# musyoku/wavenet

Hardware: AMD Instinct MI355X
Metric: audio samples/sec: train fwd+bwd, 4x10-layer dilated stack (cfg2) (higher is better)
Workload: dtype f32 storage+accumulate / fp16x2 split products (2^-21)

## Files before the change

wavenet_amd/csrc/mfma_gemm_b3.hip:

```cpp
#include "mfma_gemm.hpp"
#include "split_w.hpp"
#include "h2_ops.hpp"
#include <type_traits>

namespace wn {

template <bool WMAX>
__global__ void k_split_w(CGArgs a, int mode, int mtiles, int chunks_per_src, __bf16* __restrict__ img, int one) {
    if (WMAX) {
        const float mw = split_w_tile<true>(a, mode, mtiles, chunks_per_src, img, one, (int)blockIdx.x, 1.f);
        if (threadIdx.x == 0) atomicMax(const_cast<unsigned*>(a.wmax_dev), __float_as_uint(mw));
    } else {
        split_w_tile<false>(a, mode, mtiles, chunks_per_src, img, one, (int)blockIdx.x, one == 3 ? h2_scale(a.wmax_dev, kH2ScaleW) : 1.f);
    }
}

__device__ __forceinline__ int b3_ch(int r, int h) { return (r & 3) + 8 * (r >> 2) + 4 * h; }

struct RowMap { long long row[4]; bool ok[4]; };

__device__ __forceinline__ RowMap row_map(long long no, bool nvalid, int lane) {
    RowMap m;
#pragma unroll
    for (int it = 0; it < 4; ++it) {
// ... 421 lines not shown
    if (MODE == 3) {
        const bool live = rbase - a.off >= a.gate_Z;
#pragma unroll
        for (int pr = 0; pr < MT / 2; ++pr) {
            if (t0 + 2 * pr >= mtiles) break;
            const int col = ((t0 >> 1) + pr) * 32;
            float4 tf[4], ts[4], tz[4];
#pragma unroll
            for (int q = 0; q < 4; ++q) {
                float f4[4], s4[4];
#pragma unroll
                for (int e = 0; e < 4; ++e) {
                    f4[e] = fast_tanh(live ? acc[2 * pr][4 * q + e] : 0.f);
                    s4[e] = fast_sigmoid(live ? acc[2 * pr + 1][4 * q + e] : 0.f);
                }
                tf[q] = make_float4(f4[0], f4[1], f4[2], f4[3]);
                ts[q] = make_float4(s4[0], s4[1], s4[2], s4[3]);
                tz[q] = make_float4(f4[0] * s4[0], f4[1] * s4[1], f4[2] * s4[2], f4[3] * s4[3]);
            }
            tile_store_rows(patch, lane, tz, a.gate_z, a.M, col, rm);
            if (a.gate_f) {
                tile_store_rows(patch, lane, tf, a.gate_f, a.M, col, rm);
                tile_store_rows(patch, lane, ts, a.gate_s, a.M, col, rm);
            }
        }
        return;
    }
    if (MODE == 4) {
        const bool live = rbase - a.off >= a.gate_Z;
#pragma unroll
        for (int mt = 0; mt < MT; ++mt) {
            if (t0 + mt >= mtiles) break;
            const int col = (t0 + mt) * 32;
            float4 vf[4], vs[4], vr[4], tf[4], ts[4], tr[4], da[4], dg[4];
            rows_load(a.gate_f, a.M, col, rm, lane, vf);
            rows_load(a.gate_s, a.M, col, rm, lane, vs);
            if (a.residual) rows_load(a.residual, a.M, col, rm, lane, vr);
            rows_to_tile(patch, lane, vf, tf);
            rows_to_tile(patch, lane, vs, ts);
            if (a.residual) rows_to_tile(patch, lane, vr, tr);
#pragma unroll
            for (int q = 0; q < 4; ++q) {
                float4 dz = make_float4(acc[mt][4 * q], acc[mt][4 * q + 1], acc[mt][4 * q + 2], acc[mt][4 * q + 3]);
                if (a.residual) { dz.x += tr[q].x; dz.y += tr[q].y; dz.z += tr[q].z; dz.w += tr[q].w; }
                if (!live) dz = make_float4(0.f, 0.f, 0.f, 0.f);
                const float4 f4 = tf[q], s4 = ts[q];
                da[q] = make_float4(dz.x * s4.x * (1.f - f4.x * f4.x), dz.y * s4.y * (1.f - f4.y * f4.y),
                                    dz.z * s4.z * (1.f - f4.z * f4.z), dz.w * s4.w * (1.f - f4.w * f4.w));
                dg[q] = make_float4(dz.x * f4.x * s4.x * (1.f - s4.x), dz.y * f4.y * s4.y * (1.f - s4.y),
                                    dz.z * f4.z * s4.z * (1.f - s4.z), dz.w * f4.w * s4.w * (1.f - s4.w));
            }
            tile_store_rows(patch, lane, da, a.gate_z, 2 * a.M, col, rm);
            tile_store_rows(patch, lane, dg, a.gate_z, 2 * a.M, a.M + col, rm);
        }
        return;
    }
    float omax = 0.f;
#pragma unroll
    for (int mt = 0; mt < MT; ++mt) {
        if (t0 + mt >= mtiles) break;
        float* __restrict__ og = (MODE == 2) ? a.out[t0 + mt] : a.out[0];
        const int col = (MODE == 2) ? 0 : (t0 + mt) * 32;
        float4 t[4], v[4], u[4];
#pragma unroll
        for (int q = 0; q < 4; ++q) t[q] = make_float4(acc[mt][4 * q], acc[mt][4 * q + 1], acc[mt][4 * q + 2], acc[mt][4 * q + 3]);
        if (MODE == 0 && a.gate_x) {
            rows_load(a.gate_x, a.ldo, col, rm, lane, v);
            rows_to_tile(patch, lane, v, u);
#pragma unroll
            for (int q = 0; q < 4; ++q) {
                t[q].x *= act_grad(u[q].x, a.gate_act); t[q].y *= act_grad(u[q].y, a.gate_act);
                t[q].z *= act_grad(u[q].z, a.gate_act); t[q].w *= act_grad(u[q].w, a.gate_act);
            }
        }
        if (MODE == 0 && a.residual) {
            rows_load(a.residual, a.ldo, col, rm, lane, v);
            rows_to_tile(patch, lane, v, u);
#pragma unroll
            for (int q = 0; q < 4; ++q) { t[q].x += u[q].x; t[q].y += u[q].y; t[q].z += u[q].z; t[q].w += u[q].w; }
        }
        if (a.accumulate) {
            rows_load(og, a.ldo, col, rm, lane, v);
            rows_to_tile(patch, lane, v, u);
#pragma unroll
            for (int q = 0; q < 4; ++q) { t[q].x += u[q].x; t[q].y += u[q].y; t[q].z += u[q].z; t[q].w += u[q].w; }
        }
        if (MODE == 0 && a.outmax_dev && nvalid) {
#pragma unroll
            for (int q = 0; q < 4; ++q)
                omax = fmaxf(omax, fmaxf(fmaxf(fabsf(t[q].x), fabsf(t[q].y)), fmaxf(fabsf(t[q].z), fabsf(t[q].w))));
        }
        tile_store_rows(patch, lane, t, og, a.ldo, col, rm);
    }
    if (MODE == 0 && a.outmax_dev) {
        for (int o = 32; o >= 1; o >>= 1) omax = fmaxf(omax, __shfl_xor(omax, o));
        if (lane == 0) {
            const unsigned bits = __float_as_uint(omax);
            if (bits > __hip_atomic_load(a.outmax_dev, __ATOMIC_RELAXED, __HIP_MEMORY_SCOPE_AGENT)) atomicMax(a.outmax_dev, bits);
        }
    }
}

typedef float f32x4 __attribute__((ext_vector_type(4)));
__device__ __forceinline__ void asm_load16(f32x4& dst, const float* p) {
    asm volatile("global_load_dwordx4 %0, %1, off" : "=v"(dst) : "v"(p) : "memory");
}
static constexpr int kH2qTB = kTileBytes * 2 / 3;
static constexpr int kH2qHalf = kH2qTB / 2;
static constexpr int kH2qLds = 4 * 8 * kH2qHalf;

__device__ __forceinline__ void asm_load16s(f32x4& dst, unsigned voff, const char* sbase) {
    asm volatile("global_load_dwordx4 %0, %1, %2" : "=v"(dst) : "v"(voff), "s"(sbase) : "memory");
}
__device__ __forceinline__ void asm_dma2(unsigned voff, const char* sbase, unsigned m0v) {
    asm volatile("s_mov_b32 m0, %2\n\ts_nop 0\n\tglobal_load_lds_dwordx4 %0, %1\n\tglobal_load_lds_dwordx4 %0, %1 offset:1024"
                 :: "v"(voff), "s"(sbase), "s"(m0v) : "memory", "m0");
}

template <int MODE, int ACT>
__global__ __launch_bounds__(256, 2) void k_colgemm_h2q(CGArgs a, const __bf16* __restrict__ img, int mtiles, int nchunks,
                                                        long long x_stride) {
    constexpr int MT = 8;
    static_assert(MODE == 0 || MODE == 2, "plain contractions only");
    extern __shared__ __attribute__((aligned(16))) char ldsq[];
    const float h2sx = h2_scale(a.xmax_dev, kH2ScaleX);
    const float h2sw = h2_scale(a.wmax_dev, kH2ScaleW);
    const int tid = threadIdx.x, lane = tid & 63, wave = tid >> 6;
    const int j = lane & 31, h = lane >> 5;
    int bx, by;
    {
        const int ny = (mtiles + MT - 1) / MT;
        const int nx = gridDim.x / ny;
        const int id = blockIdx.x;
        const int full = nx & ~7;
        if (id < full * ny) {
            const int g = id / (8 * ny), rem = id - g * 8 * ny;
            bx = g * 8 + (rem & 7);
            by = rem >> 3;
        } else {
            const int t = id - full * ny;
            by = t % ny;
            bx = full + t / ny;
        }
    }
    const int t0 = by * MT;
    const long long n = ((long long)bx * 4 + wave) * 32 + j;
    const bool nvalid = n < a.N;
    long long rb0 = 0;
    int rbase = -(1 << 30);
    long long no = n;
    if (nvalid) {
        long long b = n / a.rows_out_per_b;
        rbase = (int)(n - b * a.rows_out_per_b) + a.off;
        rb0 = b * a.rows_src_per_b;
        if (a.out_rows_per_b) no = b * a.out_rows_per_b + a.out_row0 + (n - b * a.rows_out_per_b);
    }
    f32x16 acc[MT];
#pragma unroll
    for (int mt = 0; mt < MT; ++mt)
#pragma unroll
        for (int r = 0; r < 16; ++r) acc[mt][r] = 0.f;
    if (MODE == 0) {
        for (int src = 0; src < a.nsrc; ++src)
            if (a.bias[src]) {
#pragma unroll
                for (int mt = 0; mt < MT; ++mt)
                    if (t0 + mt < mtiles) {
#pragma unroll
                        for (int r = 0; r < 16; ++r) acc[mt][r] += a.bias[src][(t0 + mt) * 32 + b3_ch(r, h)] * (h2sw * h2sx);
                    }
            }
    }
    const int nhalf = 2 * nchunks;
    const unsigned lds0 = (unsigned)(unsigned long long)(__attribute__((address_space(3))) char*)ldsq;
    const int swave = __builtin_amdgcn_readfirstlane(wave);
    unsigned tile_off[2];
#pragma unroll
    for (int tt = 0; tt < 2; ++tt)
        tile_off[tt] = (unsigned)((t0 + swave + 4 * tt < mtiles) ? t0 + swave + 4 * tt : mtiles - 1) * kH2qTB + lane * 16;
    const long long img_stride = (long long)mtiles * kH2qTB;
    auto dma_half = [&](int s) {
        const int ss = s < nhalf ? s : nhalf - 1;
        const char* base = reinterpret_cast<const char*>(img) + (long long)(ss >> 1) * img_stride + (ss & 1) * kH2qHalf;
#pragma unroll
        for (int tt = 0; tt < 2; ++tt)
            asm_dma2(tile_off[tt], base, lds0 + ((s & 3) * MT + swave + 4 * tt) * kH2qHalf);
    };
    f32x4 xr[4][2];
    const int rs0 = rbase + a.soff[0];
    const bool rv0 = rs0 >= 0 && rs0 < a.rows_src_per_b;
    const float msk0 = rv0 ? 1.f : 0.f;
    const unsigned x_off = (unsigned)(((rb0 + (rv0 ? rs0 : 0)) * (a.ldx ? a.ldx : a.K[0]) + 8 * h) * 4);
    const char* x0 = reinterpret_cast<const char*>(a.X[0]);
    auto load_x = [&](int s, auto slot_tag) {
        constexpr int slot = decltype(slot_tag)::value;
        const int ss = s < nhalf ? s : nhalf - 1;
        const char* base = x0 + (long long)(ss >> 1) * x_stride + (ss & 1) * 64;
        asm_load16s(xr[slot][0], x_off, base);
        asm_load16s(xr[slot][1], x_off + 16, base);
    };
    f16x8 xh[2], xm[2];
    auto split_one = [&](const f32x4 (&raw)[2], float ms, int e, f16x8& oh, f16x8& om) {
        const float v = raw[e >> 2][e & 3];
        _Float16 a0, a1;
        split2h(act_apply_t<ACT>(v) * (ms * h2sx), a0, a1);
        oh[e] = a0; om[e] = a1;
    };
    using I0 = std::integral_constant<int, 0>;
    using I1 = std::integral_constant<int, 1>;
    using I2 = std::integral_constant<int, 2>;
    using I3 = std::integral_constant<int, 3>;
    load_x(0, I0{});
    asm volatile("s_waitcnt vmcnt(0)" : "+v"(xr[0][0]), "+v"(xr[0][1]) : : "memory");
#pragma unroll
    for (int e = 0; e < 8; ++e) split_one(xr[0], msk0, e, xh[0], xm[0]);
    asm volatile("" : "+v"(xh[0]), "+v"(xm[0]));
    dma_half(0); load_x(1, I1{});
    dma_half(1); load_x(2, I2{});
    dma_half(2); load_x(3, I3{});

    auto step = [&](int s, auto p_tag) {
        constexpr int p = decltype(p_tag)::value;
        constexpr int set = p & 1, nxt = 1 - set;
        constexpr int rn = (p + 1) & 3;
        asm volatile("s_waitcnt vmcnt(12)" : "+v"(xr[rn][0]), "+v"(xr[rn][1]) : : "memory");
        const float ms = msk0;
        asm volatile("s_waitcnt lgkmcnt(0)" ::: "memory");
        __builtin_amdgcn_s_barrier();
        dma_half(s + 3);
        const char* Ab = ldsq + (p * MT) * kH2qHalf + lane * 16;
        f16x8 fr[2][2];
        auto ldA = [&](int mt, f16x8 (&f)[2]) {
            f[0] = *reinterpret_cast<const f16x8*>(Ab + mt * kH2qHalf);
            f[1] = *reinterpret_cast<const f16x8*>(Ab + mt * kH2qHalf + 1024);
        };
        ldA(0, fr[0]);
#pragma unroll
        for (int mt = 0; mt < MT; ++mt) {
            f16x8 (&f)[2] = fr[mt & 1];
            asm volatile("" ::"v"(f[0]));
            asm volatile("" ::"v"(f[1]));
            if (mt + 1 < MT) ldA(mt + 1, fr[(mt + 1) & 1]);
            __builtin_amdgcn_sched_barrier(0);
            split_one(xr[rn], ms, mt, nxt ? xh[1] : xh[0], nxt ? xm[1] : xm[0]);
            acc[mt] = __builtin_amdgcn_mfma_f32_32x32x16_f16(f[1], xh[set], acc[mt], 0, 0, 0);
            acc[mt] = __builtin_amdgcn_mfma_f32_32x32x16_f16(f[0], xm[set], acc[mt], 0, 0, 0);
            acc[mt] = __builtin_amdgcn_mfma_f32_32x32x16_f16(f[0], xh[set], acc[mt], 0, 0, 0);
            __builtin_amdgcn_sched_barrier(0);
        }
        asm volatile("" : "+v"(xh[nxt]), "+v"(xm[nxt]));
        load_x(s + 4, p_tag);
    };
    for (int s = 0; s < nhalf; s += 4) {
        step(s, I0{});
        step(s + 1, I1{});
        step(s + 2, I2{});
        step(s + 3, I3{});
    }
    asm volatile("s_waitcnt vmcnt(0)"
                 : "+v"(xr[0][0]), "+v"(xr[0][1]), "+v"(xr[1][0]), "+v"(xr[1][1]), "+v"(xr[2][0]), "+v"(xr[2][1]),
                   "+v"(xr[3][0]), "+v"(xr[3][1])
                 :
                 : "memory");
#pragma unroll
    for (int mt = 0; mt < MT; ++mt)
#pragma unroll
        for (int r = 0; r < 16; ++r) acc[mt][r] *= 1.f / (h2sw * h2sx);
    __syncthreads();
    float* patch = reinterpret_cast<float*>(ldsq) + wave * 1024;
    const RowMap rm = row_map(no, nvalid, lane);
#pragma unroll
    for (int mt = 0; mt < MT; ++mt) {
        if (t0 + mt >= mtiles) break;
        float* __restrict__ og = (MODE == 2) ? a.out[t0 + mt] : a.out[0];
        const int col = (MODE == 2) ? 0 : (t0 + mt) * 32;
        float4 t[4], v[4], u[4];
#pragma unroll
        for (int q = 0; q < 4; ++q) t[q] = make_float4(acc[mt][4 * q], acc[mt][4 * q + 1], acc[mt][4 * q + 2], acc[mt][4 * q + 3]);
        if (MODE == 0 && a.gate_x) {
            rows_load(a.gate_x, a.ldo, col, rm, lane, v);
            rows_to_tile(patch, lane, v, u);
#pragma unroll
            for (int q = 0; q < 4; ++q) {
                t[q].x *= act_grad(u[q].x, a.gate_act); t[q].y *= act_grad(u[q].y, a.gate_act);
                t[q].z *= act_grad(u[q].z, a.gate_act); t[q].w *= act_grad(u[q].w, a.gate_act);
            }
        }
        if (MODE == 0 && a.residual) {
            rows_load(a.residual, a.ldo, col, rm, lane, v);
            rows_to_tile(patch, lane, v, u);
#pragma unroll
            for (int q = 0; q < 4; ++q) { t[q].x += u[q].x; t[q].y += u[q].y; t[q].z += u[q].z; t[q].w += u[q].w; }
        }
        if (a.accumulate) {
            rows_load(og, a.ldo, col, rm, lane, v);
            rows_to_tile(patch, lane, v, u);
#pragma unroll
            for (int q = 0; q < 4; ++q) { t[q].x += u[q].x; t[q].y += u[q].y; t[q].z += u[q].z; t[q].w += u[q].w; }
        }
        tile_store_rows(patch, lane, t, og, a.ldo, col, rm);
    }
}

int launch_colgemm_b3(Call& c, CGArgs& a, int mode, int nprob, hipStream_t s) {
    if (mode != 0 && mode != 2 && mode != 3 && mode != 4 && mode != 5 && mode != 6) return WN_ESHAPE;
    if (mode == 6 && !(c.fp16x2() && a.M == 256 && a.nsrc == 1 && a.xent_target && a.xent_loss && a.out[0] &&
                       cdiv(a.N, 128) <= kXentBlocks))
        return WN_ESHAPE;
    int mtiles, nchunks, cps;
    if (mode == 0 || mode >= 3) {
        if (a.M % 32) return WN_ESHAPE;
        if ((mode == 3 || mode == 5) && a.nsrc > WN_GATE_TAPS) return WN_ESHAPE;
        if (mode == 5 && !(c.one_term() && a.M == 128 && a.ldo == 128)) return WN_ESHAPE;
        for (int i = 0; i < a.nsrc; ++i)
            if (a.K[i] != a.K[0] || a.K[i] % 32) return WN_ESHAPE;
        mtiles = ((mode == 3 || mode == 5) ? 2 : 1) * a.M / 32;
        cps = a.K[0] / 32;
        nchunks = a.nsrc * cps;
    } else {
        if (a.M != 32 || a.K[0] % 32) return WN_ESHAPE;
        mtiles = nprob;
        cps = a.K[0] / 32;
        nchunks = cps;
    }
    const bool one = c.one_term();
    const bool h2 = c.fp16x2() && ((a.h2_ok || a.xmax_dev) && (mode == 0 || mode == 2) || mode == 6);
    const size_t bytes = (size_t)nchunks * mtiles * (one ? kTileBytes / 3 : (h2 ? kTileBytes * 2 / 3 : kTileBytes));
    const size_t bytes2 = mode == 5 ? (size_t)16 * (kTileBytes / 3) : 0;
    const __bf16* pimg = nullptr; const unsigned* pwmax = nullptr;
    const bool planned = plan_split_image(c, a, mode, mtiles, cps, nchunks, one ? 1 : (h2 ? 3 : 0), bytes, &pimg, &pwmax);
    __bf16* img = planned ? const_cast<__bf16*>(pimg)
                          : reinterpret_cast<__bf16*>(c.scratch(bytes + bytes2, "the split weight image"));
    if (!img) return WN_EARG;
    if (planned) {
        a.wmax_dev = pwmax;
    } else {
    if (h2) {
        bool fresh = false;
        unsigned* wm = c.word(reinterpret_cast<const char*>(a.W[0]) + (((unsigned)mode & 7u) << 8 | ((unsigned)a.nsrc & 255u)), &fresh, s);
        if (!wm) return WN_EARG;
        a.wmax_dev = wm;
        if (fresh) hipLaunchKernelGGL(k_split_w<true>, dim3(nchunks * mtiles), dim3(256), 0, s, a, mode, mtiles, cps, img, 3);
    }
    hipLaunchKernelGGL(k_split_w<false>, dim3(nchunks * mtiles), dim3(256), 0, s, a, mode, mtiles, cps, img, one ? 1 : (h2 ? 3 : 0));
    }
    if (mode == 5) {
        if (!a.proj_W || !a.residual || !a.gate_z || a.act != WN_ACT_NONE || mtiles != 8) {
            wn::set_error("colgemm_b3: fused-layer mode needs Wp, the residual input, z and 128 gate channels");
            return WN_EARG;
        }
        CGArgs b{};
        b.nsrc = 1; b.W[0] = a.proj_W; b.wsm[0] = 128; b.wsk = 1; b.K[0] = 128; b.M = 128;
        __bf16* img2 = reinterpret_cast<__bf16*>(reinterpret_cast<char*>(img) + bytes);
        hipLaunchKernelGGL(k_split_w<false>, dim3(16), dim3(256), 0, s, b, 0, 4, 4, img2, 1);
        hipLaunchKernelGGL((k_colgemm_b3<5, WN_ACT_NONE, 1, 8>), dim3(cdiv(a.N, 128)), dim3(256), 0, s, a,
                           (const __bf16*)img, mtiles, nchunks, cps, (const __bf16*)img2);
        WN_LAUNCH_CHECK();
        return WN_OK;
    }
    const bool mt8 = (one || h2) && mtiles >= 8;
    dim3 grid(cdiv(a.N, 128) * cdiv(mtiles, mt8 ? 8 : 4));
    if (mode == 6) {
#define X_LAUNCH(ACT_, ROWS_) hipLaunchKernelGGL((k_colgemm_b3<6, ACT_, 3, 8, ROWS_>), grid, dim3(256), 0, s, a, (const __bf16*)img, \
                                                 mtiles, nchunks, cps, (const __bf16*)nullptr)
        if (c.flag(WN_EXEC_HEAD_ROW_NLL)) {
            if (a.act == WN_ACT_RELU) X_LAUNCH(WN_ACT_RELU, true);
            else if (a.act == WN_ACT_ELU) X_LAUNCH(WN_ACT_ELU, true);
            else X_LAUNCH(WN_ACT_NONE, true);
        } else if (a.act == WN_ACT_RELU) X_LAUNCH(WN_ACT_RELU, false);
        else if (a.act == WN_ACT_ELU) X_LAUNCH(WN_ACT_ELU, false);
        else X_LAUNCH(WN_ACT_NONE, false);
#undef X_LAUNCH
        WN_LAUNCH_CHECK();
        return WN_OK;
    }
#define CG_LAUNCH(MODE_, ACT_)                                                                                          \
    do {                                                                                                                \
        if (mt8) hipLaunchKernelGGL((k_colgemm_b3<MODE_, ACT_, 1, 8>), grid, dim3(256), 0, s, a, (const __bf16*)img,    \
                                    mtiles, nchunks, cps, (const __bf16*)nullptr);                                      \
        else if (one) hipLaunchKernelGGL((k_colgemm_b3<MODE_, ACT_, 1, 4>), grid, dim3(256), 0, s, a,                   \
                                         (const __bf16*)img, mtiles, nchunks, cps, (const __bf16*)nullptr);             \
        else hipLaunchKernelGGL((k_colgemm_b3<MODE_, ACT_, 6, 4>), grid, dim3(256), 0, s, a, (const __bf16*)img,        \
                                mtiles, nchunks, cps, (const __bf16*)nullptr);                                          \
    } while (0)
#define CG_LAUNCH_H2(MODE_, ACT_)                                                                                       \
    do {                                                                                                                \
        if (mt8) hipLaunchKernelGGL((k_colgemm_b3<MODE_, ACT_, 3, 8>), grid, dim3(256), 0, s, a, (const __bf16*)img,    \
                                    mtiles, nchunks, cps, (const __bf16*)nullptr);                                      \
        else hipLaunchKernelGGL((k_colgemm_b3<MODE_, ACT_, 3, 4>), grid, dim3(256), 0, s, a, (const __bf16*)img,        \
                                mtiles, nchunks, cps, (const __bf16*)nullptr);                                          \
    } while (0)
    long long x_stride = 128;
    bool lean = h2 && mt8 && mode == 0 && (nchunks & 1) == 0 && !c.flag(WN_EXEC_NO_PIPELINED_GEMM) &&
                (a.N / a.rows_out_per_b + 1) * (long long)a.rows_src_per_b * (a.ldx ? a.ldx : a.K[0]) * 4 < (1ll << 32);
    if (lean && mode == 0 && a.nsrc > 1) {
        x_stride = (const char*)a.X[1] - (const char*)a.X[0];
        lean = cps == 1;
        for (int i = 1; i < a.nsrc && lean; ++i)
            lean = a.soff[i] == a.soff[0] && a.K[i] == a.K[0] && (const char*)a.X[i] - (const char*)a.X[i - 1] == x_stride;
    } else if (lean && mode == 0) {
        lean = a.nsrc == 1;
    }
    if (lean) {
        WN_MAX_LDS_ONCE(kH2qLds, k_colgemm_h2q<0, WN_ACT_NONE>, k_colgemm_h2q<0, WN_ACT_RELU>, k_colgemm_h2q<0, WN_ACT_ELU>);
#define Q_LAUNCH(MODE_, ACT_)                                                                                 \
    hipLaunchKernelGGL((k_colgemm_h2q<MODE_, ACT_>), grid, dim3(256), kH2qLds, s, a, (const __bf16*)img, mtiles, nchunks, x_stride)
        if (a.act == WN_ACT_RELU) Q_LAUNCH(0, WN_ACT_RELU);
        else if (a.act == WN_ACT_ELU) Q_LAUNCH(0, WN_ACT_ELU);
        else Q_LAUNCH(0, WN_ACT_NONE);
#undef Q_LAUNCH
        WN_LAUNCH_CHECK();
        return WN_OK;
    }
    if (h2) {
        if (mode == 2) CG_LAUNCH_H2(2, WN_ACT_NONE);
        else if (a.act == WN_ACT_RELU) CG_LAUNCH_H2(0, WN_ACT_RELU);
        else if (a.act == WN_ACT_ELU) CG_LAUNCH_H2(0, WN_ACT_ELU);
        else CG_LAUNCH_H2(0, WN_ACT_NONE);
        WN_LAUNCH_CHECK();
        return WN_OK;
    }
#undef CG_LAUNCH_H2
    if (mode == 3) {
        if (a.act != WN_ACT_NONE || !a.gate_z) { wn::set_error("colgemm_b3: gate mode takes no activation and needs gate_z"); return WN_EARG; }
        CG_LAUNCH(3, WN_ACT_NONE);
    } else if (mode == 4) {
        if (a.act != WN_ACT_NONE || !a.gate_z || !a.gate_f || !a.gate_s) { wn::set_error("colgemm_b3: gate-backward mode needs f, s and the output"); return WN_EARG; }
        CG_LAUNCH(4, WN_ACT_NONE);
    } else if (mode == 0) {
        if (a.outmax_dev) plan_xmax_written(c, a.out[0]);
        if (a.act == WN_ACT_RELU) CG_LAUNCH(0, WN_ACT_RELU);
        else if (a.act == WN_ACT_ELU) CG_LAUNCH(0, WN_ACT_ELU);
        else if (a.act == WN_ACT_NONE) CG_LAUNCH(0, WN_ACT_NONE);
        else { wn::set_error("colgemm_b3: unknown activation %d", a.act); return WN_EARG; }
    } else {
        if (a.act != WN_ACT_NONE) { wn::set_error("colgemm_b3: multi-problem mode takes no activation"); return WN_EARG; }
        CG_LAUNCH(2, WN_ACT_NONE);
    }
#undef CG_LAUNCH
    WN_LAUNCH_CHECK();
    return WN_OK;
}

template <int MT, bool HAS_B2, int ACT, bool ONE>
__global__ __launch_bounds__(256, 2) void k_wgrad_b3(WGArgs a) {
    __shared__ __attribute__((aligned(16))) char lds[MT * kTileBytes];
    constexpr int NF = MT / 2 > 0 ? MT / 2 : 1;
    const int tid = threadIdx.x, lane = tid & 63, wv = tid >> 6;
    const int j = lane & 31, h = lane >> 5;
    const int p = blockIdx.y * 4 + wv;
    const bool active = p < a.nprob;
    const int m0 = blockIdx.z * (MT * 32);
    const int b = blockIdx.x / a.wgs_per_b;
    const int r_begin = (blockIdx.x - b * a.wgs_per_b) * a.rows_per_wg;
    const int r_end = min(a.rows_A_per_b, r_begin + a.rows_per_wg);
    const float* __restrict__ Ab = a.A + ((long long)b * a.rows_A_per_b) * a.lda + m0;
    const float* __restrict__ Bb = a.Bp[active ? p : 0] + ((long long)b * a.rows_B_per_b + a.off) * a.ldb + j;
    const float* __restrict__ B2b = a.B2p[active ? p : 0] ? a.B2p[active ? p : 0] + ((long long)b * a.rows_B_per_b + a.off) * a.ldb + j : nullptr;
    f32x16 acc[MT];
#pragma unroll
    for (int mt = 0; mt < MT; ++mt)
#pragma unroll
        for (int r = 0; r < 16; ++r) acc[mt][r] = 0.f;

    float ar[NF][8], br[2][8], b2r[2][8];
    const float* __restrict__ B2s = HAS_B2 ? B2b : Bb;
    const float amask = active ? 1.f : 0.f;
    int fm[NF], fg[NF];
#pragma unroll
    for (int it = 0; it < NF; ++it) {
        const int f = it * 256 + tid;
        fm[it] = f % (MT * 32);
        fg[it] = f / (MT * 32);
    }
    auto issue = [&](int r0) {
        const bool full = r0 + 32 <= r_end && r0 + a.off >= 0 && r0 + 31 + a.off < a.rows_B_per_b;
        if (full) {
#pragma unroll
            for (int it = 0; it < NF; ++it) {
                const float* ap = Ab + (long long)(r0 + 8 * (fg[it] & 3)) * a.lda + fm[it];
#pragma unroll
                for (int jj = 0; jj < 8; ++jj) ar[it][jj] = ap[(long long)jj * a.lda];
            }
            const float* bp = Bb + (long long)(r0 + 8 * h) * a.ldb;
            const float* b2p = B2s + (long long)(r0 + 8 * h) * a.ldb;
#pragma unroll
            for (int ks = 0; ks < 2; ++ks)
#pragma unroll
                for (int jj = 0; jj < 8; ++jj) {
                    br[ks][jj] = bp[(long long)(16 * ks + jj) * a.ldb];
                    if (HAS_B2) b2r[ks][jj] = b2p[(long long)(16 * ks + jj) * a.ldb];
                }
            return;
        }
#pragma unroll
        for (int it = 0; it < NF; ++it)
#pragma unroll
            for (int jj = 0; jj < 8; ++jj) {
                const int r = r0 + 8 * (fg[it] & 3) + jj;
                const int rc = r < r_end ? r : r_end - 1;
                ar[it][jj] = Ab[(long long)rc * a.lda + fm[it]];
            }
#pragma unroll
        for (int ks = 0; ks < 2; ++ks)
#pragma unroll
            for (int jj = 0; jj < 8; ++jj) {
                const int r = r0 + 16 * ks + 8 * h + jj;
                int rc = r < r_end ? r : r_end - 1;
                if (rc + a.off < 0) rc = -a.off;
                if (rc + a.off >= a.rows_B_per_b) rc = a.rows_B_per_b - 1 - a.off;
                br[ks][jj] = Bb[(long long)rc * a.ldb];
                if (HAS_B2) b2r[ks][jj] = B2s[(long long)rc * a.ldb];
            }
    };
    if (r_begin < r_end) issue(r_begin);
    for (int r0 = r_begin; r0 < r_end; r0 += 32) {
        bf16x8 ah[NF], am[NF], al[NF], bh[2], bm[2], bl[2];
        const bool edge = !(r0 + 32 <= r_end && r0 + a.off >= 0 && r0 + 31 + a.off < a.rows_B_per_b);
#pragma unroll
        for (int it = 0; it < NF; ++it)
#pragma unroll
            for (int e = 0; e < 8; ++e) {
                float av = ar[it][e];
                if (edge) av *= (r0 + 8 * (fg[it] & 3) + e) < r_end ? 1.f : 0.f;
                __bf16 x0, x1, x2;
                split3(av, x0, x1, x2);
                ah[it][e] = x0; am[it][e] = x1; al[it][e] = x2;
            }
#pragma unroll
        for (int ks = 0; ks < 2; ++ks)
#pragma unroll
            for (int e = 0; e < 8; ++e) {
                float bv = act_apply_t<ACT>(br[ks][e]) * amask;
                if (HAS_B2) bv *= b2r[ks][e];
                if (edge) {
                    const int rb = r0 + 16 * ks + 8 * h + e;
                    bv *= (rb < r_end && rb + a.off >= 0 && rb + a.off < a.rows_B_per_b) ? 1.f : 0.f;
                }
                __bf16 x0, x1, x2;
                split3(bv, x0, x1, x2);
                bh[ks][e] = x0; bm[ks][e] = x1; bl[ks][e] = x2;
            }
        __syncthreads();
#pragma unroll
        for (int it = 0; it < NF; ++it) {
            const int f = it * 256 + tid;
            const int m = f % (MT * 32), g = f / (MT * 32);
            if (MT >= 2 || g < 4) {
                char* d = lds + (m >> 5) * kTileBytes + ((g >> 1) * 3) * 1024 + ((m & 31) + 32 * (g & 1)) * 16;
                *reinterpret_cast<bf16x8*>(d) = ah[it];
                *reinterpret_cast<bf16x8*>(d + 1024) = am[it];
                *reinterpret_cast<bf16x8*>(d + 2048) = al[it];
            }
        }
        __syncthreads();
        if (r0 + 32 < r_end) issue(r0 + 32);
        const char* Al = lds + lane * 16;
#pragma unroll
        for (int mt = 0; mt < MT; ++mt) {
#pragma unroll
            for (int ks = 0; ks < 2; ++ks) {
                const char* q = Al + mt * kTileBytes + ks * 3 * 1024;
                const bf16x8 xh = *reinterpret_cast<const bf16x8*>(q);
                const bf16x8 xm = *reinterpret_cast<const bf16x8*>(q + 1024);
                const bf16x8 xl = *reinterpret_cast<const bf16x8*>(q + 2048);
                if (!ONE) {
                    acc[mt] = __builtin_amdgcn_mfma_f32_32x32x16_bf16(xl, bh[ks], acc[mt], 0, 0, 0);
                    acc[mt] = __builtin_amdgcn_mfma_f32_32x32x16_bf16(xh, bl[ks], acc[mt], 0, 0, 0);
                    acc[mt] = __builtin_amdgcn_mfma_f32_32x32x16_bf16(xm, bm[ks], acc[mt], 0, 0, 0);
                    acc[mt] = __builtin_amdgcn_mfma_f32_32x32x16_bf16(xm, bh[ks], acc[mt], 0, 0, 0);
                    acc[mt] = __builtin_amdgcn_mfma_f32_32x32x16_bf16(xh, bm[ks], acc[mt], 0, 0, 0);
                }
                acc[mt] = __builtin_amdgcn_mfma_f32_32x32x16_bf16(xh, bh[ks], acc[mt], 0, 0, 0);
            }
        }
    }
    if (!active) return;
    if (a.fixed_part) {
        const long long M = (long long)gridDim.z * (MT * 32);
        float* __restrict__ q = a.fixed_part + (((long long)blockIdx.x * a.nprob + p) * M) * 32 + j;
#pragma unroll
        for (int mt = 0; mt < MT; ++mt)
#pragma unroll
            for (int r = 0; r < 16; ++r) q[(long long)(m0 + mt * 32 + b3_ch(r, h)) * 32] = acc[mt][r];
        return;
    }
    float* __restrict__ o = a.out[p];
#pragma unroll
    for (int mt = 0; mt < MT; ++mt)
#pragma unroll
        for (int r = 0; r < 16; ++r)
            atomicAdd(o + (long long)(m0 + mt * 32 + b3_ch(r, h)) * a.ldo + (long long)j * (a.osk ? a.osk : 1), acc[mt][r]);
}

template <bool HAS_B2, int ACT, int TM>
__global__ __launch_bounds__(512, 1) void k_wgrad_b3w(WGArgs a) {
    constexpr int MT = 8;
    constexpr bool ONE = TM == 1;
    constexpr bool H2 = TM == 3;
    const float h2sa = H2 ? h2_scale(a.amax_dev, 1.f) : 1.f;
    const float h2sb = H2 ? h2_scale(a.bmax_dev, kH2ScaleX) : 1.f;
    extern __shared__ __attribute__((aligned(16))) char ldsw[];
    const int tid = threadIdx.x, lane = tid & 63, wv = tid >> 6;
    const int j = lane & 31, h = lane >> 5;
    const int p = blockIdx.y * 8 + wv;
    const bool active = p < a.nprob;
    const int off = a.off + a.offp[active ? p : 0];
    const int b = blockIdx.x / a.wgs_per_b;
    const int r_begin = (blockIdx.x - b * a.wgs_per_b) * a.rows_per_wg;
    const int r_end = min(a.rows_A_per_b, r_begin + a.rows_per_wg);
    const float* __restrict__ Ab = a.A + ((long long)b * a.rows_A_per_b) * a.lda;
    const float* __restrict__ Bb = a.Bp[active ? p : 0] + ((long long)b * a.rows_B_per_b + off) * a.ldb + j;
    const float* __restrict__ B2b = a.B2p[active ? p : 0] ? a.B2p[active ? p : 0] + ((long long)b * a.rows_B_per_b + off) * a.ldb + j : nullptr;
    f32x16 acc[MT];
#pragma unroll
    for (int mt = 0; mt < MT; ++mt)
#pragma unroll
        for (int r = 0; r < 16; ++r) acc[mt][r] = 0.f;

    const int fm = tid & 255;
    const int fhh = tid >> 8;
    float ar[2][8], br[2][8], b2r[2][8];
    const float* __restrict__ B2s = HAS_B2 ? B2b : Bb;
    auto issue = [&](int r0) {
        const bool full = r0 + 32 <= r_end && r0 + off >= 0 && r0 + 31 + off < a.rows_B_per_b;
        if (full) {
#pragma unroll
            for (int ks = 0; ks < 2; ++ks) {
                const float* ap = Ab + (long long)(r0 + 16 * ks + 8 * fhh) * a.lda + fm;
#pragma unroll
                for (int jj = 0; jj < 8; ++jj) ar[ks][jj] = ap[(long long)jj * a.lda];
            }
            const float* bp = Bb + (long long)(r0 + 8 * h) * a.ldb;
            const float* b2p = B2s + (long long)(r0 + 8 * h) * a.ldb;
#pragma unroll
            for (int ks = 0; ks < 2; ++ks)
#pragma unroll
                for (int jj = 0; jj < 8; ++jj) {
                    br[ks][jj] = bp[(long long)(16 * ks + jj) * a.ldb];
                    if (HAS_B2) b2r[ks][jj] = b2p[(long long)(16 * ks + jj) * a.ldb];
                }
            return;
        }
#pragma unroll
        for (int ks = 0; ks < 2; ++ks)
#pragma unroll
            for (int jj = 0; jj < 8; ++jj) {
                const int r = r0 + 16 * ks + 8 * fhh + jj;
                const int rc = r < r_end ? r : r_end - 1;
                ar[ks][jj] = Ab[(long long)rc * a.lda + fm];
            }
#pragma unroll
        for (int ks = 0; ks < 2; ++ks)
#pragma unroll
            for (int jj = 0; jj < 8; ++jj) {
                const int r = r0 + 16 * ks + 8 * h + jj;
                int rc = r < r_end ? r : r_end - 1;
                if (rc + off < 0) rc = -off;
                if (rc + off >= a.rows_B_per_b) rc = a.rows_B_per_b - 1 - off;
                br[ks][jj] = Bb[(long long)rc * a.ldb];
                if (HAS_B2) b2r[ks][jj] = B2s[(long long)rc * a.ldb];
// ... 385 lines not shown
```

Measured before the change: 47.53 million.

## Add persistent weight-stationary pipelined kernel for mode-2 fp16x2 dz GEMM

Adds a persistent kernel for the mode-2 fp16x2 GEMM with 8 chunks and ldo 32. Each wave keeps its layer's split weight fragments in registers, and the block walks a contiguous range of 32-column tiles. Within a step it double-buffers the split X tile in LDS and overlaps the next tile's global load, split and store with the current tile's MFMAs. The grid is sized to device occupancy, which aims to cut repeated weight loads and launch and tail overhead. It costs a large register footprint at one block per CU and a more complex schedule built on sched barriers.

```diff
diff --git a/wavenet_amd/csrc/mfma_gemm_b3.hip b/wavenet_amd/csrc/mfma_gemm_b3.hip
--- a/wavenet_amd/csrc/mfma_gemm_b3.hip
+++ b/wavenet_amd/csrc/mfma_gemm_b3.hip
@@ -747,6 +747,185 @@
     }
 }
 
+static constexpr int kWsTile = 32 * 1024;
+static constexpr int kWsLds = 2 * kWsTile + 8 * 4096;
+static constexpr int kWsAhead = 2;
+
+__global__ __launch_bounds__(512, 1) void k_dz_ws(CGArgs a, const __bf16* __restrict__ img, int mtiles, int ntiles, int nranges) {
+    extern __shared__ __attribute__((aligned(16))) char ldsw[];
+    const float h2sx = h2_scale(a.xmax_dev, kH2ScaleX);
+    const float h2sw = h2_scale(a.wmax_dev, kH2ScaleW);
+    const int tid = threadIdx.x, lane = tid & 63;
+    const int wave = __builtin_amdgcn_readfirstlane(tid >> 6);
+    const int j = lane & 31, h = lane >> 5;
+    int range, grp;
+    {
+        const int ng = (mtiles + 7) >> 3;
+        const int id = blockIdx.x;
+        const int full = nranges & ~7;
+        if (id < full * ng) {
+            const int g = id / (8 * ng), rem = id - g * 8 * ng;
+            range = g * 8 + (rem & 7);
+            grp = rem >> 3;
+        } else {
+            const int t = id - full * ng;
+            grp = t % ng;
+            range = full + t / ng;
+        }
+    }
+    const int t_lo = (int)((long long)range * ntiles / nranges), t_hi = (int)((long long)(range + 1) * ntiles / nranges);
+    if (t_lo >= t_hi) return;
+    const int layer = grp * 8 + wave;
+    const bool live = layer < mtiles;
+    const int N = (int)a.N, rows_out = a.rows_out_per_b, rows_src = a.rows_src_per_b, shift = a.off + a.soff[0];
+    const int ldo = a.ldo;
+    const long long ldx = a.ldx ? a.ldx : a.K[0];
+    const float* __restrict__ X = a.X[0];
+    float* __restrict__ og = a.out[live ? layer : 0];
+
+    f16x8 A[16][2];
+    {
+        const char* ip = reinterpret_cast<const char*>(img) + (long long)(live ? layer : mtiles - 1) * kH2qTB + lane * 16;
+#pragma unroll
+        for (int kk = 0; kk < 16; ++kk)
+#pragma unroll
+            for (int pl = 0; pl < 2; ++pl)
+                A[kk][pl] = *reinterpret_cast<const f16x8*>(ip + (long long)(kk >> 1) * mtiles * kH2qTB + (kk & 1) * kH2qHalf + pl * 1024);
+    }
+
+    auto advance = [&](int& n, int& b, int& r, int by) {
+        n += by; r += by;
+        const bool wrap = r >= rows_out;
+        r -= wrap ? rows_out : 0;
+        b += wrap ? 1 : 0;
+    };
+    const int lcol = (tid & 7) | ((tid >> 7) << 3), kseg = (tid >> 3) & 15;
+    int ln = t_lo * 32 + lcol, lb = ln / rows_out, lr = ln - lb * rows_out;
+    float4 raw[4];
+    float rsc = 0.f;
+    auto load_raw = [&]() {
+        const int rs = lr + shift;
+        const bool rv = ln < N && rs >= 0 && rs < rows_src;
+        rsc = rv ? h2sx : 0.f;
+        const float* p = X + (rv ? (long long)lb * rows_src + rs : 0ll) * ldx + 16 * kseg;
+#pragma unroll
+        for (int i = 0; i < 4; ++i) raw[i] = reinterpret_cast<const float4*>(p)[i];
+        advance(ln, lb, lr, 32);
+    };
+    auto split_write = [&](char* buf) {
+        float v[16];
+#pragma unroll
+        for (int e = 0; e < 16; ++e) {
+            const float x = (e & 3) == 0 ? raw[e >> 2].x : (e & 3) == 1 ? raw[e >> 2].y : (e & 3) == 2 ? raw[e >> 2].z : raw[e >> 2].w;
+            v[e] = fminf(fmaxf(x * rsc, -65000.f), 65000.f);
+        }
+        H2Op o;
+        lb_split16(v, 1.f, o);
+        char* d = buf + kseg * 2048 + lcol * 16;
+        *reinterpret_cast<f16x8*>(d) = o.h[0];
+        *reinterpret_cast<f16x8*>(d + 512) = o.h[1];
+        *reinterpret_cast<f16x8*>(d + 1024) = o.m[0];
+        *reinterpret_cast<f16x8*>(d + 1536) = o.m[1];
+    };
+    float* patch = reinterpret_cast<float*>(ldsw + 2 * kWsTile) + wave * 1024;
+    const int orows = a.out_rows_per_b ? a.out_rows_per_b : rows_out, orow0 = a.out_rows_per_b ? a.out_row0 : 0;
+    int sn[4], sb[4], sr[4];
+#pragma unroll
+    for (int it = 0; it < 4; ++it) {
+        sn[it] = t_lo * 32 + it * 8 + (lane >> 3);
+        sb[it] = sn[it] / rows_out;
+        sr[it] = sn[it] - sb[it] * rows_out;
+    }
+    float4 pv0, pv1, pv2, pv3;
+    auto patch_read = [&]() {
+        pv0 = *reinterpret_cast<const float4*>(patch_rows(patch, lane, 0));
+        pv1 = *reinterpret_cast<const float4*>(patch_rows(patch, lane, 1));
+        pv2 = *reinterpret_cast<const float4*>(patch_rows(patch, lane, 2));
+        pv3 = *reinterpret_cast<const float4*>(patch_rows(patch, lane, 3));
+    };
+    auto store_rows = [&](const float4 v, int& n, int& b, int& r, bool en) {
+        const long long no = (long long)b * orows + orow0 + r;
+        if (en && n < N) *reinterpret_cast<float4*>(og + no * ldo + ((lane & 7) << 2)) = v;
+        advance(n, b, r, en ? 32 : 0);
+    };
+    auto store_tile = [&](bool en) {
+        store_rows(pv0, sn[0], sb[0], sr[0], en);
+        store_rows(pv1, sn[1], sb[1], sr[1], en);
+        store_rows(pv2, sn[2], sb[2], sr[2], en);
+        store_rows(pv3, sn[3], sb[3], sr[3], en);
+    };
+
+    f32x16 acc;
+#pragma unroll
+    for (int r = 0; r < 16; ++r) acc[r] = 0.f;
+    const float inv = 1.f / (h2sw * h2sx);
+
+    auto step = [&](auto live_tag, int t) {
+        constexpr bool LIVE = decltype(live_tag)::value;
+        char* nxt = ldsw + ((t - t_lo + 1) & 1) * kWsTile;
+        const char* rd = ldsw + ((t - t_lo) & 1) * kWsTile + lane * 16;
+        f16x8 fr[kWsAhead + 1][2];
+        auto ldB = [&](int kk, f16x8 (&f)[2]) {
+            f[0] = *reinterpret_cast<const f16x8*>(rd + kk * 2048);
+            f[1] = *reinterpret_cast<const f16x8*>(rd + kk * 2048 + 1024);
+        };
+        if (LIVE) {
+#pragma unroll
+            for (int kk = 0; kk < kWsAhead; ++kk) ldB(kk, fr[kk]);
+        }
+#pragma unroll
+        for (int kk = 0; kk < 16; ++kk) {
+            if (LIVE) {
+                f16x8 (&f)[2] = fr[kk % (kWsAhead + 1)];
+                asm volatile("" ::"v"(f[0]));
+                asm volatile("" ::"v"(f[1]));
+                if (kk + kWsAhead < 16) ldB(kk + kWsAhead, fr[(kk + kWsAhead) % (kWsAhead + 1)]);
+                __builtin_amdgcn_sched_barrier(0);
+                acc = __builtin_amdgcn_mfma_f32_32x32x16_f16(A[kk][1], f[0], acc, 0, 0, 0);
+                acc = __builtin_amdgcn_mfma_f32_32x32x16_f16(A[kk][0], f[1], acc, 0, 0, 0);
+                acc = __builtin_amdgcn_mfma_f32_32x32x16_f16(A[kk][0], f[0], acc, 0, 0, 0);
+                __builtin_amdgcn_sched_barrier(0);
+            }
+            if (kk == 5) {
+                split_write(nxt);
+                __builtin_amdgcn_sched_barrier(0);
+            }
+            if (kk == 6 && LIVE) {
+                patch_read();
+                __builtin_amdgcn_sched_barrier(0);
+            }
+            if (kk == 7) {
+                if (LIVE) store_tile(t > t_lo);
+                load_raw();
+                __builtin_amdgcn_sched_barrier(0);
+            }
+        }
+        if (LIVE) {
+#pragma unroll
+            for (int q = 0; q < 4; ++q)
+                *reinterpret_cast<float4*>(patch_tile(patch, j, h, q)) =
+                    make_float4(acc[4 * q] * inv, acc[4 * q + 1] * inv, acc[4 * q + 2] * inv, acc[4 * q + 3] * inv);
+#pragma unroll
+            for (int r = 0; r < 16; ++r) acc[r] = 0.f;
+        }
+        asm volatile("s_waitcnt lgkmcnt(0)" ::: "memory");
+        __builtin_amdgcn_s_barrier();
+    };
+
+    load_raw();
+    split_write(ldsw);
+    load_raw();
+    asm volatile("s_waitcnt lgkmcnt(0)" ::: "memory");
+    __builtin_amdgcn_s_barrier();
+    if (live) {
+        for (int t = t_lo; t < t_hi; ++t) step(std::true_type{}, t);
+        patch_read();
+        store_tile(true);
+    } else {
+        for (int t = t_lo; t < t_hi; ++t) step(std::false_type{}, t);
+    }
+}
+
 int launch_colgemm_b3(Call& c, CGArgs& a, int mode, int nprob, hipStream_t s) {
     if (mode != 0 && mode != 2 && mode != 3 && mode != 4 && mode != 5 && mode != 6) return WN_ESHAPE;
     if (mode == 6 && !(c.fp16x2() && a.M == 256 && a.nsrc == 1 && a.xent_target && a.xent_loss && a.out[0] &&
@@ -802,6 +981,29 @@
                            (const __bf16*)img, mtiles, nchunks, cps, (const __bf16*)img2);
         WN_LAUNCH_CHECK();
         return WN_OK;
+    }
+    if (h2 && mode == 2 && nchunks == 8 && a.ldo == 32 && !a.accumulate && !c.flag(WN_EXEC_NO_PIPELINED_GEMM) &&
+        a.N < (1ll << 30) && a.rows_out_per_b >= 32 &&
+        (a.N / a.rows_out_per_b + 2) * (long long)(a.out_rows_per_b > a.rows_out_per_b ? a.out_rows_per_b : a.rows_out_per_b) < (1ll << 31)) {
+        int dev = 0;
+        WN_HIP(hipGetDevice(&dev));
+        static int capacity[64];
+        if (dev < 0 || dev >= 64) { wn::set_error("colgemm_b3: device index %d", dev); return WN_ESHAPE; }
+        if (!capacity[dev]) {
+            int n_cu = 0, per_cu = 0;
+            WN_HIP(hipDeviceGetAttribute(&n_cu, hipDeviceAttributeMultiprocessorCount, dev));
+            WN_HIP(hipFuncSetAttribute(reinterpret_cast<const void*>(k_dz_ws), hipFuncAttributeMaxDynamicSharedMemorySize, kWsLds));
+            WN_HIP(hipOccupancyMaxActiveBlocksPerMultiprocessor(&per_cu, k_dz_ws, 512, kWsLds));
+            capacity[dev] = n_cu * per_cu > 0 ? n_cu * per_cu : -1;
+        }
+        const int ng = cdiv(mtiles, 8), ntiles = cdiv(a.N, 32);
+        int nranges = capacity[dev] / ng;
+        if (nranges > ntiles) nranges = ntiles;
+        if (nranges >= 1) {
+            hipLaunchKernelGGL(k_dz_ws, dim3(ng * nranges), dim3(512), kWsLds, s, a, (const __bf16*)img, mtiles, ntiles, nranges);
+            WN_LAUNCH_CHECK();
+            return WN_OK;
+        }
     }
     const bool mt8 = (one || h2) && mtiles >= 8;
     dim3 grid(cdiv(a.N, 128) * cdiv(mtiles, mt8 ? 8 : 4));
```

Measured after the change: 48.02 million (median of 6 runs). 1.01x the previous value.
